# lajoiepy/cslam

Hardware: AMD Instinct MI355X
Metric: keyframes/sec (extract+match) on 100kx4096-D bank (higher is better)
Workload: dtype f32

## Files before the change

### cslam_amd/_lib.py

```python
import ctypes as C
import os
import subprocess

_HERE = os.path.dirname(os.path.abspath(__file__))
LIB_PATH = os.environ.get("CSLAM_HIP_LIB") or os.path.join(_HERE, "libcslam_hip.so")
CSRC_DIR = os.path.join(_HERE, "csrc")

F32, F64 = 0, 1
MODE_AUTO, MODE_SCAN, MODE_MFMA = 0, 1, 2


class CslamHipError(RuntimeError):
    pass


class CslamGraphError(CslamHipError):
    """CSLAM_E_GRAPH: the graph admits no Fiedler pair (not connected, singular junction Laplacian, TraceMIN breakdown) --
    the condition under which the reference's networkx call raises and acm.py:436-466 re-draws its start point.  Not a
    failure of the GPU path."""


class CslamUnsupportedError(CslamHipError):
    """CSLAM_E_UNSUPPORTED: an optional run-time dependency (RCCL, rocBLAS / rocSOLVER) was not found on this host."""

# ... 9 lines not shown
_vp, _i, _i64, _f = C.c_void_p, C.c_int, C.c_int64, C.c_float
_SIGNATURES = {
    "cslam_last_error": (C.c_char_p, []),
    "cslam_version": (_i, []),
    "cslam_device_count": (_i, [C.POINTER(_i)]),
    "cslam_device_info": (_i, [_i, C.c_char_p, _i, C.POINTER(_i64), C.POINTER(_i)]),
    "cslam_bank_create": (_i, [_i, _i, _i64, C.POINTER(_vp)]),
    "cslam_bank_destroy": (_i, [_vp]),
    "cslam_bank_size": (_i, [_vp, C.POINTER(_i64), C.POINTER(_i)]),
    "cslam_bank_clear": (_i, [_vp]),
    "cslam_bank_add_host": (_i, [_vp, _vp, _i, _i64]),
    "cslam_bank_add_dev": (_i, [_vp, _vp, _i64, _i64, _vp]),
    "cslam_bank_read_host": (_i, [_vp, _i64, _i64, _vp]),
    "cslam_bank_device_ptr": (_i, [_vp, C.POINTER(_vp), C.POINTER(_i64)]),
    "cslam_bank_search_host": (_i, [_vp, _vp, _i, _i64, _i, _vp, _i, _vp, _vp, _vp]),
    "cslam_bank_search_dev": (_i, [_vp, _vp, _i, _i64, _i64, _i, _vp, _i, _vp, _vp, _vp, _vp]),
    "cslam_bank_search_multi_dev": (_i, [_vp, _i, _vp, _i, _i64, _i64, _vp, _vp, _i, _vp, _vp, _vp, _vp]),
    "cslam_bank_search_enqueue_dev": (_i, [_vp, _vp, _i, _i64, _i64, _i, _vp, _i, _vp, _vp, _vp, _vp]),
    "cslam_bank_search_finish": (_i, [_vp, C.POINTER(_i64)]),
    "cslam_bank_search_flag_copy_dev": (_i, [_vp, _vp, _vp]),
    "cslam_bank_search_multi_enqueue_dev": (_i, [_vp, _i, _vp, _i, _i64, _i64, _vp, _vp, _i, _vp, _vp, _vp, _vp]),
    "cslam_bank_search_multi_finish": (_i, [_vp, _i, C.POINTER(_i64)]),
    "cslam_bank_last_stats": (_i, [_vp, C.POINTER(_i64 * 4)]),
    "cslam_bank_last_stage": (_i, [_vp, C.POINTER(C.c_int32 * 4)]),
    "cslam_bank_last_kernel_ms": (_i, [_vp, C.POINTER(_f)]),
    "cslam_topk_merge_dev": (_i, [_vp, _vp, _vp, _vp, _i, _i64, _i, _vp, _vp, _vp, _vp]),
    "cslam_l2_normalize_dev": (_i, [_vp, _i64, _i, _i64, _f, _i, _vp]),
    "cslam_vlad_aggregate_dev": (_i, [_vp, _vp, _vp, _vp, _i, _i, _i, _i, _vp, _i64, _vp]),
    "cslam_vlad_aggregate_nhwc_dev": (_i, [_vp, _vp, _vp, _vp, _i, _i, _i, _i, _vp, _i64, _vp]),
    "cslam_gem_fc_head_dev": (_i, [_vp, _f, _f, _vp, _vp, _i, _i, _i, _i, _vp, _vp]),
    "cslam_gem_fc_head_nhwc_dev": (_i, [_vp, _f, _f, _vp, _vp, _i, _i, _i, _i, _vp, _vp]),
    "cslam_pca_project_dev": (_i, [_vp, _i64, _vp, _i64, _vp, _vp, _i, _i, _i, _vp, _vp]),
    "cslam_pca_project_pairs_dev": (_i, [_vp, _i64, C.c_float, _vp, C.c_float, _i, _vp, _vp, _i, _i, _i, _vp, _vp]),
    "cslam_preprocess_dev": (_i, [_vp, _i, _i, _i, _i, _i, C.POINTER(_f * 3), C.POINTER(_f * 3), _vp, _vp]),
    "cslam_preprocess_nhwc_dev": (_i, [_vp, _i, _i, _i, _i, _i, C.POINTER(_f * 3), C.POINTER(_f * 3), _vp, _vp]),
    "cslam_mac_grad_dev": (_i, [_vp, _vp, _vp, _vp, _i64, _vp, _vp]),
    "cslam_csr_spmm_dev": (_i, [_vp, _vp, _vp, _i64, _vp, _i, _vp, _vp]),
    "cslam_csr_spmm4_dev": (_i, [_vp, _vp, _vp, _i64, _vp, _vp, _vp]),
    "cslam_block4_gram_dev": (_i, [_vp, _vp, _i64, _vp, _vp, _vp]),
    "cslam_block4_affine_dev": (_i, [_vp, _i64, _vp, _vp, _vp, _vp]),
    "cslam_block4_residual_dev": (_i, [_vp, _vp, _i64, _vp, C.c_double, _vp, _vp, _vp]),
    "cslam_block4_gram_sync": (_i, [_vp, _vp, _i64, _vp, _vp, _vp, _vp]),
    "cslam_block4_affine_host": (_i, [_vp, _i64, _vp, _vp, _vp, _vp]),
    "cslam_block4_residual_sync": (_i, [_vp, _vp, _i64, _vp, C.c_double, _vp, _vp, _vp, _vp]),
    "cslam_chain_forward_dev": (_i, [_vp, _vp, _vp, _i64, _vp, _i, _vp, _vp, _vp, _vp, _vp, _vp, _vp, _vp, _vp, _vp, _vp]),
    "cslam_chain_backward_dev": (_i, [_vp, _vp, _vp, _vp, _vp, _vp, _vp, _vp, _vp, _vp, _i64, _vp, _vp]),
    "cslam_chol_solve4_dev": (_i, [_vp, _i64, _i64, _i, _vp, _vp, _i, _vp, _vp, _vp]),
    "cslam_fiedler": (_i, [_i64, _vp, _vp, _vp, _vp, C.c_uint32, C.c_double, _i, _vp, _vp, _vp, _vp]),
    "cslam_fiedler_start_block": (_i, [C.c_uint32, _i64, _vp]),
    "cslam_fiedler_release": (_i, []),
    "cslam_mac_fw_subset": (_i, [_i64, _i64, _vp, _vp, _vp, _i64, _vp, _vp, _vp, _vp, _i64, _i, C.c_double, C.c_double, _vp, _vp, _vp, _vp, _vp]),
    "cslam_scbank_create": (_i, [_i, _i, _i, _i64, _vp]),
    "cslam_scbank_destroy": (_i, [_vp]),
    "cslam_scbank_size": (_i, [_vp, _vp, _vp, _vp]),
    "cslam_scbank_clear": (_i, [_vp]),
    "cslam_scbank_add_host": (_i, [_vp, _vp, _i64]),
    "cslam_scbank_add_dev": (_i, [_vp, _vp, _i64, _vp]),
    "cslam_scbank_read_host": (_i, [_vp, _i64, _i64, _vp, _vp]),
    "cslam_scbank_search_host": (_i, [_vp, _vp, _i64, _i, _vp, _vp, _vp, _vp, _vp, _vp, _vp]),
    "cslam_scbank_search_dev": (_i, [_vp, _vp, _i64, _i, _vp, _vp, _vp, _vp, _vp, _vp, _vp, _vp]),
    "cslam_bias_act_pool_dev": (_i, [_vp, _vp, _i, _i, _i, _i, _i, _i, _vp, _vp]),
    "cslam_conv3x3_c3_dev": (_i, [_vp, _vp, _vp, _i, _i, _i, _i, _i, _vp, _vp]),
    "cslam_wino_input_dev": (_i, [_vp, _i, _i, _i, _i, _vp, _vp]),
    "cslam_wino_output_dev": (_i, [_vp, _vp, _vp, _i, _i, _i, _i, _i, _i, _vp, _vp]),
    "cslam_wino4_input_dev": (_i, [_vp, _i, _i, _i, _i, _vp, _vp]),
    "cslam_wino4_output_dev": (_i, [_vp, _vp, _vp, _i, _i, _i, _i, _i, _i, _vp, _vp]),
    "cslam_absmax_dev": (_i, [_vp, _i64, _vp, _vp]),
    "cslam_wino4_input_h3_dev": (_i, [_vp, _i, _i, _i, _i, _vp, _vp, _vp]),
    "cslam_wino4_output_scaled_dev": (_i, [_vp, _vp, _vp, _i, _i, _i, _i, _i, _i, _vp, C.c_float, _vp, _vp, _vp]),
    "cslam_wino2_fused64_dev": (_i, [_vp, _vp, _vp, _i, _i, _i, _i, _i, _vp, _vp]),
    "cslam_wino2_fused_c64_dev": (_i, [_vp, _vp, _vp, _vp, _i, _i, _i, _i, _i, _i, _vp, _vp]),
    "cslam_wino4_fused_c64_dev": (_i, [_vp, _vp, _vp, _vp, _i, _i, _i, _i, _i, _i, _vp, _vp]),
    "cslam_scancontext_from_cloud_dev": (_i, [_vp, _vp, _i, _i, _i, C.c_double, _vp, _vp, _vp]),
    "cslam_wino4_fused_c64_h_dev": (_i, [_vp, _vp, _vp, _vp, _i, _i, _i, _i, _i, _i, _vp, C.c_float, _vp, _vp, _vp]),
    "cslam_conv3x3_direct_h_dev": (_i, [_vp, _vp, _vp, _i, _i, _i, _i, _i, _i, _i, _vp, _f, _vp, _vp, _vp]),
    "cslam_conv3x3_direct_r_dev": (_i, [_vp, _vp, _vp, _i, _i, _i, _i, _i, _i, _i, _vp, C.c_float, _vp, _vp, _vp]),
    "cslam_conv3x3_direct_r2_dev": (_i, [_vp, _vp, _vp, _i, _i, _i, _i, _i, _i, _i, _vp, C.c_float, _vp, _vp, _vp]),
    "cslam_conv_stem_direct_h_dev": (_i, [_vp, _vp, _vp, _vp, C.c_float, _vp, _vp, C.c_float, _i, _i, _i, _i, _vp, _vp, _vp, _vp]),
    "cslam_wino4_stem_c64_h_dev": (_i, [_vp, _vp, _vp, _vp, C.c_float, _vp, _vp, _i, _i, _i, _i, _vp, C.c_float, _vp, _vp, _vp]),
    "cslam_debug_wfh_prof_dev": (_i, [_vp]),
    "cslam_conv3x3_c3_amax_dev": (_i, [_vp, _vp, _vp, _i, _i, _i, _i, _i, _vp, _vp, _vp]),
    "cslam_wino4_input_h2_dev": (_i, [_vp, _i, _i, _i, _i, _vp, _vp, _vp]),
    "cslam_wino_gemm_h2_dev": (_i, [_vp, _vp, _i64, _i, _i, _vp, _vp]),
    "cslam_wino_zgemm_h2_dev": (_i, [_vp, _vp, _i64, _i, _i, _vp, _vp]),
    "cslam_wino4_output_z_dev": (_i, [_vp, _vp, _i, _i, _i, _i, _i, _i, _vp, C.c_float, _vp, _vp, _vp]),
    "cslam_conv_igemm_h2_dev": (_i, [_vp, _vp, _vp, _vp, _i, _i, _i, _i, _i, _i, _i, _i, _i, _i, _vp, C.c_float, _vp, _vp, _vp]),
    "cslam_conv_stem_pool_igemm_h2_dev": (_i, [_vp, _vp, _vp, _i, _i, _i, _i, _i, _i, _i, _i, _vp, C.c_float, _vp, _vp, _vp]),
    "cslam_conv_igemm_h2p_dev": (_i, [_vp, _i, _vp, _vp, _vp, _vp, _i, _vp, _i, _i, _i, _i, _i, _i, _i, _i, _i, _i, _vp, C.c_float,
                                      C.c_float, C.c_float, _vp, _i, _vp, _vp, _vp]),
    "cslam_conv3x3_direct_r_pairs_dev": (_i, [_vp, _vp, _vp, _i, _i, _i, _i, _i, _vp, C.c_float, C.c_float, C.c_float, _vp, _vp, _vp, _vp]),
    "cslam_conv3x3_direct_hp_dev": (_i, [_vp, _vp, _vp, _vp, _i, _i, _i, _i, _i, _i, _i, C.c_float, _vp, _vp, _vp]),
    "cslam_conv3x3_direct_p_dev": (_i, [_vp, _i, _vp, _vp, _vp, _vp, _i, _vp, _i, _i, _i, _i, _i, _i, _vp, C.c_float, C.c_float, C.c_float,
                                        _vp, _i, _vp, _vp, _vp]),
    "cslam_comm_unique_id": (_i, [_vp]),
    "cslam_comm_init": (_i, [_i, _i, _vp, _i, C.POINTER(_vp)]),
    "cslam_comm_destroy": (_i, [_vp]),
    "cslam_comm_info": (_i, [_vp, C.POINTER(_i), C.POINTER(_i)]),
    "cslam_allgather_queries_dev": (_i, [_vp, _vp, _i64, _i64, _vp, _vp]),
    "cslam_exchange_lists_dev": (_i, [_vp, _vp, _vp, _i64, _vp]),
    "cslam_peak_copy_dev": (_i, [_vp, _vp, _i64, _i, _vp]),
    "cslam_peak_mfma_dev": (_i, [_i, _i, _i, _i, _vp, C.POINTER(C.c_double), _vp]),
    "cslam_debug_last_candidates": (_i, [_vp, _i64, C.POINTER(_i), _vp, _vp, C.POINTER(C.c_double)]),
    "cslam_ring_schedule_describe": (_i, [_i, _i, _i, _i, C.POINTER(C.c_int32 * 6), _vp, _i64, _vp, _vp, _vp]),
    "cslam_trunk_timing": (_i, [_i]),
    "cslam_trunk_timing_read": (_i, [C.POINTER(C.c_double * 8)]),
}

EXPERIMENTAL_SYMBOLS = ("cslam_wino4_input_h3_dev", "cslam_wino2_fused64_dev", "cslam_wino2_fused_c64_dev",
                        "cslam_wino4_fused_c64_dev", "cslam_debug_wfh_prof_dev", "cslam_peak_copy_dev", "cslam_peak_mfma_dev",
                        "cslam_debug_last_candidates", "cslam_ring_schedule_describe", "cslam_trunk_timing", "cslam_trunk_timing_read")
EXPORTED_SYMBOLS = tuple(n for n in _SIGNATURES if n not in EXPERIMENTAL_SYMBOLS)


def build(verbose=False):
    r = subprocess.run(["make", "-C", CSRC_DIR, "-j", "4"], capture_output=True, text=True)
    if verbose or r.returncode != 0:
        print(r.stdout[-4000:])
        print(r.stderr[-4000:])
    if r.returncode != 0:
        raise CslamHipError("building libcslam_hip.so failed")
    return LIB_PATH


def load():
    global _lib
    if _lib is not None:
        return _lib
    try:
        import torch
    except ImportError:
        pass
    if not os.path.exists(LIB_PATH):
        raise CslamHipError(
            f"{LIB_PATH} not found: the HIP extension is not built "
            "(run `python __graft_entry__.py` or `make -C cslam_amd/csrc`); there is no CPU fallback")
    lib = C.CDLL(LIB_PATH)
    for name, (res, args) in _SIGNATURES.items():
        fn = getattr(lib, name)
        fn.restype = res
        fn.argtypes = args
    _lib = lib
    return lib


def check(rc):
    if rc != 0:
        msg = load().cslam_last_error()
        raise _ERROR_CLASSES.get(rc, CslamHipError)(f"libcslam_hip error {rc}: {msg.decode() if msg else ''}")


def require_gpu():
    lib = load()
    n = C.c_int(0)
    rc = lib.cslam_device_count(C.byref(n))
    if rc != 0 or n.value < 1:
        msg = lib.cslam_last_error()
        raise CslamHipError("no HIP device visible: cslam_amd needs an MI355X (gfx950); "
                            f"no CPU fallback exists ({msg.decode() if msg else ''})")
    return n.value
```

### cslam_amd/vpr/winograd.py

```python
import ctypes as C
import os

import torch
from torch import nn

from .. import _lib
from .heads import _p, _stream, pair_split

_G = torch.tensor([[1.0, 0.0, 0.0], [0.5, 0.5, 0.5], [0.5, -0.5, 0.5], [0.0, 0.0, 1.0]], dtype=torch.float64)
_G4 = torch.tensor([[1 / 4, 0.0, 0.0], [-1 / 6, -1 / 6, -1 / 6], [-1 / 6, 1 / 6, -1 / 6],
                    [1 / 24, 1 / 12, 1 / 6], [1 / 24, -1 / 12, 1 / 6], [0.0, 0.0, 1.0]], dtype=torch.float64)


def wino_weights(weight, tile=2):
    G = _G if tile == 2 else _G4
    g = weight.detach().to(torch.float64).cpu()
    u = torch.einsum("ik,ockl,jl->ijco", G, g, G)
    return u.reshape(G.shape[0] ** 2, g.shape[1], g.shape[0]).to(torch.float32).contiguous()


def split16_weights(U4):
    u = U4.detach().to(torch.float64)
    uh, ul, inv_su = pair_split(u)
    return torch.cat((uh, uh, ul), dim=1).contiguous(), inv_su
# ... 512 lines not shown
                self.blocks.append(d)
        return self

    @torch.no_grad()
    def __call__(self, x, x_bound=None):
        x = x.contiguous(memory_format=torch.channels_last)
        slots = self._buf("amax_slots", 4 * len(self.blocks) + 6, x.device)
        slots.zero_()
        nslot = [0]

        def fresh():
            nslot[0] += 1
            return slots[nslot[0] - 1:nslot[0]]

        def run(conv, inp, relu, res, a_in):
            out_slot = fresh()
            y = conv(self, inp, relu, res, a_in, out_slot)
            return y, (out_slot if self.amax_written else None)
        a0 = None
        if x_bound is not None:
            a0 = fresh()
            a0.fill_(float(x_bound))
        sp = self.stem_pool
        ho = (x.shape[2] + 2 * self.stem.padding[0] - self.stem.kernel[0]) // self.stem.stride[0] + 1
        wo = (x.shape[3] + 2 * self.stem.padding[1] - self.stem.kernel[1]) // self.stem.stride[1] + 1
        if (self.stem.Wg is not None and x.shape[1] == 3 and stem_pool_fits(ho, wo) and isinstance(sp, torch.nn.MaxPool2d)
                and _pair(sp.kernel_size) == (3, 3) and _pair(sp.stride) == (2, 2) and _pair(sp.padding) == (1, 1)
                and _pair(sp.dilation) == (1, 1) and not sp.ceil_mode):
            out_slot = fresh()
            x = self.stem(self, x, True, None, a0, out_slot, pool=True)
            ax = out_slot
        else:
            y, ax = run(self.stem, x, True, None, a0)
            x = sp(y)
        convs = [c for b in self.blocks for c in (b["down"], b["c1"], b["c2"], b["c3"]) if c is not None]
        if PAIR_ACTS and ax is not None and all(c.Wg is not None and c.in_channels % 32 == 0 for c in convs):
            pslots = self._buf("pair_slots", 2 * len(convs) + 2, x.device)
            pslots.zero_()
            np_ = [0]
            last = convs[-1]

            def runp(conv, a, relu, res):
                np_[0] += 2
                if (conv.Wp is not None and (a.pairs or res is None) and conv is not last
                        and direct_p_fits(conv.weight.shape, conv.kernel, conv.stride[0], conv.padding[0], a.shape[2], a.shape[3])):
                    return conv3x3_direct_p(a, conv.Wp, conv.bias, relu, res, conv.wl1, conv.bmax, pslots[np_[0] - 2:np_[0] - 1],
                                            pslots[np_[0] - 1:np_[0]], True)
                return conv_igemm_p(self, a, conv.Wg, conv.bias, conv.kernel, conv.stride[0], conv.padding[0], relu, res, conv.wl1,
                                    conv.bmax, pslots[np_[0] - 2:np_[0] - 1], pslots[np_[0] - 1:np_[0]], conv is not last)
            cur = PairAct(x, False, x.shape, ax, ax)
            for b in self.blocks:
                idt = cur if b["down"] is None else runp(b["down"], cur, False, None)
                o = runp(b["c1"], cur, True, None)
                if b["c3"] is None:
                    cur = runp(b["c2"], o, True, idt)
                else:
                    o = runp(b["c2"], o, True, None)
                    cur = runp(b["c3"], o, True, idt)
            return cur.t
        for b in self.blocks:
            idt = x if b["down"] is None else run(b["down"], x, False, None, ax)[0]
            o, ao = run(b["c1"], x, True, None, ax)
            if b["c3"] is None:
                x, ax = run(b["c2"], o, True, idt, ao)
            else:
                o, ao = run(b["c2"], o, True, None, ao)
                x, ax = run(b["c3"], o, True, idt, ao)
        return x


class _Step(object):
    __slots__ = ("kind", "module", "conv", "relu", "pool", "U", "U4", "U3", "U2", "Up", "Uph", "bias", "stem", "Wd", "Wr", "Wdr", "Wdr2", "wl1", "bmax")

    def __init__(self):
        self.kind, self.module, self.conv, self.relu, self.pool = "torch", None, None, False, False
        self.U, self.U4, self.U3, self.U2, self.Up, self.Uph, self.bias, self.stem = None, None, None, None, None, None, None, None
        self.Wd = None
        self.Wr = None
        self.Wdr = None
        self.Wdr2 = None
        self.wl1 = self.bmax = None


TRUNK_FORMS = {"conv_direct": 1, "conv_direct_r": True, "conv_direct_r2": True, "stem_direct": True, "wino_stem": True, "fused_h": True, "split16_min_cin": None}
FP32_GEMM_FORMS = {"split16_min_cin": 0, "fused_h": False, "wino_stem": False}


class WinogradTrunk(_Workspace):

    def __init__(self, encoder, min_in_channels=256, tile=2, fused64=None, split16_h3=False, forms=None):
        super().__init__()
        self.encoder = encoder
        self.min_in_channels = int(min_in_channels)
        self.tile = int(tile)
        self.fused64 = True if fused64 is None else bool(fused64)
        self.fused_min_blocks = 256
        self.fused_couts = (64, 128)
        self.input_bound = None
        self.forms = dict(TRUNK_FORMS)
        self.forms.update(forms or {})
        assert set(self.forms) == set(TRUNK_FORMS), "unknown trunk form"
        self.direct128 = int(self.forms["conv_direct"]) != 0
        self.direct_cins = (128,) if int(self.forms["conv_direct"]) == 2 else (64, 128)
        self.split16_h3 = bool(split16_h3)
        self.split16_min_cin = (256 if self.split16_h3 else 128) if self.forms["split16_min_cin"] is None else int(self.forms["split16_min_cin"])
        use_tuned_gemms()
        self.refresh()

    def refresh(self):
        mods = list(self.encoder)
        self.steps = []
        i = 0
        while i < len(mods):
            m = mods[i]
            st = _Step()
            ok = (isinstance(m, nn.Conv2d) and m.kernel_size == (3, 3) and m.stride == (1, 1) and m.padding == (1, 1)
                  and m.dilation == (1, 1) and m.groups == 1 and m.in_channels >= self.min_in_channels
                  and m.in_channels % 4 == 0 and m.out_channels % 4 == 0 and m.weight.is_cuda)
            if ok:
                st.kind, st.conv, st.relu, st.pool = "wino", m, False, False
                st.U = wino_weights(m.weight).to(m.weight.device)
                st.U4 = wino_weights(m.weight, 4).to(m.weight.device) if self.tile == 4 else None
                if st.U4 is not None and 0 < self.split16_min_cin <= m.in_channels:
                    if not self.split16_h3 and m.in_channels % 32 == 0 and m.out_channels % 128 == 0:
                        st.U2 = split16_pair_weights(st.U4)
                    else:
                        st.U3 = split16_weights(st.U4)
                if self.fused64 and m.in_channels == 64 and m.out_channels in self.fused_couts:
                    t4 = self.tile == 4
                    st.Up = fused64_weights(st.U4 if t4 else st.U)
                    if t4 and self.forms["fused_h"]:
                        st.Uph = fused64_pair_weights(st.U4)
                if (self.direct128 and self.tile == 4 and m.out_channels == 128 and m.in_channels in self.direct_cins):
                    st.Wd = direct_pair_weights(m.weight)
                    if m.in_channels == 64 and self.forms["conv_direct_r"]:
                        st.Wdr = direct_r_pair_weights(m.weight)
                        st.wl1 = float(m.weight.detach().abs().sum(dim=(1, 2, 3)).max())
                        st.bmax = 0.0 if m.bias is None else float(m.bias.detach().abs().max())
                    if m.in_channels == 128 and self.forms.get("conv_direct_r2", True):
                        st.Wdr2 = direct_r2_pair_weights(m.weight)
                st.bias = None if m.bias is None else m.bias.detach().to(torch.float32).contiguous()
                i += 1
                if i < len(mods) and isinstance(mods[i], nn.ReLU):
                    st.relu = True
                    i += 1
                    p = mods[i] if i < len(mods) else None
                    if isinstance(p, nn.MaxPool2d) and p.kernel_size in (2, (2, 2)) and p.stride in (2, (2, 2)) \
                            and p.padding in (0, (0, 0)) and not p.ceil_mode:
                        st.pool = True
                        i += 1
            elif (isinstance(m, nn.Conv2d) and m.in_channels == 3 and m.kernel_size == (3, 3) and m.stride == (1, 1)
                  and m.padding == (1, 1) and m.dilation == (1, 1) and m.groups == 1 and m.out_channels % 16 == 0
                  and m.out_channels <= 512 and m.weight.is_cuda and not (i + 2 < len(mods) and isinstance(
                      mods[i + 1], nn.ReLU) and isinstance(mods[i + 2], nn.MaxPool2d))):
                st.kind, st.conv = "c3", m
                st.U = m.weight.detach().to(torch.float32).permute(1, 2, 3, 0).reshape(27, m.out_channels).contiguous()
                st.bias = None if m.bias is None else m.bias.detach().to(torch.float32).contiguous()
                i += 1
                if i < len(mods) and isinstance(mods[i], nn.ReLU):
                    st.relu = True
                    i += 1
            elif (isinstance(m, nn.Conv2d) and m.groups == 1 and m.out_channels % 4 == 0 and m.bias is not None
                  and m.weight.is_cuda and i + 1 < len(mods) and isinstance(mods[i + 1], nn.ReLU)):
                st.kind, st.conv, st.relu = "direct", m, True
                st.bias = m.bias.detach().to(torch.float32).contiguous()
                i += 2
                p = mods[i] if i < len(mods) else None
                if isinstance(p, nn.MaxPool2d) and p.kernel_size in (2, (2, 2)) and p.stride in (2, (2, 2)) \
                        and p.padding in (0, (0, 0)) and not p.ceil_mode:
                    st.pool = True
                    i += 1
            else:
                st.kind, st.module = "torch", m
                i += 1
            self.steps.append(st)
        if self.forms["wino_stem"]:
            for a, b in zip(self.steps, self.steps[1:]):
                if (a.kind == "c3" and a.relu and a.conv.out_channels == 64 and b.kind == "wino" and b.Uph is not None
                        and b.relu and b.conv.out_channels == 64):
                    a.stem = stem_pair_weights(a.conv.weight)
                    if self.forms["stem_direct"]:
                        a.Wr = stem_direct_pair_weights(b.conv.weight)
        return self

    @torch.no_grad()
    def __call__(self, x):
        lib = _lib.load()
        slots = amax_ready = None
        wants = lambda st_: st_ is not None and (st_.U3 is not None or st_.U2 is not None or st_.Uph is not None or st_.Wd is not None)
        if any(wants(st) for st in self.steps):
            slots = self._buf("amax_slots", len(self.steps) + 1, x.device)
            slots.zero_()
        skip = False
        for k, st in enumerate(self.steps):
            if skip:
                skip = False
                continue
            have, amax_ready = amax_ready, None
            nxt = self.steps[k + 1] if k + 1 < len(self.steps) else None
            if st.kind == "c3":
                x = x.contiguous()
                B, _, H, W = x.shape
                if (st.stem is not None and B * -(-H // 16) * -(-W // 16) >= self.fused_min_blocks
                        and not (nxt.pool and (H % 2 or W % 2)) and B * H * W * 64 < 2 ** 31):
                    slot = slots[k:k + 1]
                    if self.input_bound is not None:
                        slot.fill_(float(self.input_bound))
                    elif x.numel() % 4 == 0:
                        _lib.check(lib.cslam_absmax_dev(_p(x), x.numel(), _p(slot), _stream(x)))
                    else:
                        slot.copy_(x.abs().max().reshape(1))
                    nn2 = self.steps[k + 2] if k + 2 < len(self.steps) else None
                    want = slots[k + 2:k + 3] if wants(nn2) else None
                    if st.Wr is not None:
                        x = conv_stem_direct_h(x, st.stem, st.bias, st.Wr, nxt.bias, nxt.pool, slot, want)
                    else:
                        x = wino_stem64_h(x, st.stem, st.bias, nxt.Uph, nxt.bias, nxt.pool, slot, want)
                    amax_ready = want is not None
                    skip = True
                    continue
                Cout = st.conv.out_channels
                y = torch.empty((B, Cout, H, W), dtype=torch.float32, device=x.device, memory_format=torch.channels_last)
                want = slots[k + 1:k + 2] if (wants(nxt) and Cout == 64) else None
                _lib.check(lib.cslam_conv3x3_c3_amax_dev(_p(x), _p(st.U), _p(st.bias) if st.bias is not None else None,
                                                         B, H, W, Cout, int(st.relu), _p(y),
                                                         _p(want) if want is not None else None, _stream(x)))
                amax_ready = want is not None
                x = y
                continue
            x = x.contiguous(memory_format=torch.channels_last)
            if st.kind == "torch":
                x = st.module(x)
                continue
            if st.kind == "direct":
                c = st.conv
                x = torch.nn.functional.conv2d(x, c.weight, None, c.stride, c.padding, c.dilation)
                x = x.contiguous(memory_format=torch.channels_last)
                B, Cout, H, W = x.shape
                pool = st.pool and H % 2 == 0 and W % 2 == 0
                y = x if not pool else torch.empty((B, Cout, H // 2, W // 2), dtype=torch.float32, device=x.device,
                                                   memory_format=torch.channels_last)
                _lib.check(lib.cslam_bias_act_pool_dev(_p(x), _p(st.bias), B, H, W, Cout, 1, int(pool), _p(y), _stream(x)))
                x = y if not (st.pool and not pool) else torch.nn.functional.max_pool2d(y, 2, 2)
                continue
            x = x.contiguous(memory_format=torch.channels_last)
            if (st.Wd is not None and not (st.pool and (x.shape[2] % 2 or x.shape[3] % 2))
                    and x.shape[0] * -(-x.shape[2] // 16) * -(-x.shape[3] // 16) >= self.fused_min_blocks and x.numel() % 4 == 0):
                slot = slots[k:k + 1]
                if not have:
                    _lib.check(lib.cslam_absmax_dev(_p(x), x.numel(), _p(slot), _stream(x)))
                want = slots[k + 1:k + 2] if wants(nxt) else None
                if (VGG_PAIRS and st.Wdr is not None and st.relu and not st.pool and nxt is not None and nxt.Wd is not None
                        and nxt.Wdr is None and nxt.conv.in_channels == 128 and x.shape[2] * x.shape[3] * 512 < 2 ** 31 - 16
                        and not (nxt.pool and (x.shape[2] % 2 or x.shape[3] % 2))):
                    B_, _, H_, W_ = x.shape
                    bslot = self._buf("vgg_pair_bound", 1, x.device)
                    w_ = st.conv.weight.detach()
                    xp = conv3x3_direct_r_pairs(x, st.Wdr, st.bias, float(w_.abs().sum(dim=(1, 2, 3)).max()) if st.wl1 is None else st.wl1,
                                                0.0 if st.bias is None else st.bmax, slot, bslot)
                    nn2 = self.steps[k + 2] if k + 2 < len(self.steps) else None
                    want2 = slots[k + 2:k + 3] if wants(nn2) else None
                    x = conv3x3_direct_hp(xp, (B_, 128, H_, W_), bslot, nxt.Wd, nxt.bias, nxt.relu, nxt.pool, want2)
                    amax_ready = want2 is not None
                    skip = True
                    continue
                if st.Wdr is not None and x.shape[2] * x.shape[3] * 512 < 2 ** 31 - 16:
                    x = conv3x3_direct_r(x, st.Wdr, st.bias, st.relu, st.pool, slot, want)
                elif st.Wdr2 is not None and x.shape[2] * x.shape[3] * 512 < 2 ** 31 - 16:
                    x = conv3x3_direct_r2(x, st.Wdr2, st.bias, st.relu, st.pool, slot, want)
                else:
                    x = conv3x3_direct_h(x, st.Wd, st.bias, st.relu, st.pool, slot, want)
                amax_ready = want is not None
                continue
            if st.Up is not None and not (st.pool and (x.shape[2] % 2 or x.shape[3] % 2)):
                bh, bw = (16, 16) if st.Up.shape[1] == 36 else (8, 16)
                nblk = x.shape[0] * -(-x.shape[2] // bh) * -(-x.shape[3] // bw) * st.Up.shape[2] // 4
                if nblk >= self.fused_min_blocks:
                    if st.Uph is not None and x.numel() < 2 ** 31:
                        slot = slots[k:k + 1]
                        if not have:
                            _lib.check(lib.cslam_absmax_dev(_p(x), x.numel(), _p(slot), _stream(x)))
                        want = slots[k + 1:k + 2] if wants(nxt) else None
                        x = wino_fused64_h(x, st.Uph, st.bias, st.relu, st.pool, slot, want)
                        amax_ready = want is not None
                    else:
                        x = wino_fused64(x, st.Up, st.bias, st.relu, st.pool)
                    continue
            want = slots[k + 1:k + 2] if wants(nxt) else None
            y = wino_conv3x3(self, x, st.U, st.U4, st.bias, st.relu, st.pool, U3=st.U3, U2=st.U2,
                             amax_in=slots[k:k + 1] if have else None, amax_out=want)
            amax_ready = want is not None and self.amax_written
            x = y
        return x
```

### include/cslam_hip.h

```cpp
#ifndef CSLAM_HIP_H
#define CSLAM_HIP_H

#include <stdint.h>

#ifdef __cplusplus
extern "C" {
#endif

#define CSLAM_OK 0
#define CSLAM_E_INVALID (-1)
#define CSLAM_E_HIP (-2)
#define CSLAM_E_NOMEM (-3)
#define CSLAM_E_DIM (-4)
#define CSLAM_E_UNSUPPORTED (-5)
#define CSLAM_E_GRAPH (-6)
#define CSLAM_E_LIMIT (-7)

#define CSLAM_F32 0
#define CSLAM_F64 1

#define CSLAM_MODE_AUTO 0
#define CSLAM_MODE_SCAN 1
#define CSLAM_MODE_MFMA 2

// ... 70 lines not shown

int cslam_mac_grad_dev(const double *d_fiedler, const int32_t *d_edge_i, const int32_t *d_edge_j,
                       const double *d_weights, int64_t m, double *d_grad, void *stream);
int cslam_csr_spmm_dev(const int64_t *d_indptr, const int32_t *d_indices, const double *d_data,
                       int64_t n, const double *d_x, int nvec, double *d_y, void *stream);

int cslam_csr_spmm4_dev(const int64_t *d_indptr, const int32_t *d_indices, const double *d_data,
                        int64_t n, const double *d_x, double *d_y, void *stream);

int cslam_block4_gram_dev(const double *d_A, const double *d_B, int64_t n, double *d_partial,
                          double *d_out20, void *stream);
int cslam_block4_affine_dev(const double *d_A, int64_t n, const double *d_M16, const double *d_shift4,
                            double *d_out, void *stream);
int cslam_block4_residual_dev(const double *d_W, const double *d_X, int64_t n, const double *d_y4,
                              double sigma, double *d_partial, double *d_out1, void *stream);

int cslam_block4_gram_sync(const double *d_A, const double *d_B, int64_t n, double *d_partial, double *d_out20,
                           double *h_out20, void *stream);
int cslam_block4_affine_host(const double *d_A, int64_t n, const double *h_M16, const double *h_shift4, double *d_out,
                             void *stream);
int cslam_block4_residual_sync(const double *d_W, const double *d_X, int64_t n, const double *h_y4, double sigma,
                               double *d_partial, double *d_out1, double *h_out1, void *stream);

int cslam_chain_forward_dev(const double *d_b, const uint8_t *d_is_junction, const double *d_r, int64_t n,
                            const int64_t *d_J, int nJ, const int *d_seg_start_of, const int *d_seg_end_of,
                            const int64_t *d_sa, const int64_t *d_sb, const double *d_Rl,
                            double *d_Bn, double *d_Qn, double *d_tmp, double *d_scratch, double *d_bt,
                            void *stream);
int cslam_chain_backward_dev(const double *d_xJ, const double *d_Bn, const double *d_Qn, const double *d_r,
                             const double *d_Rn, const int *d_jid, const int *d_seg_of, const int64_t *d_sa,
                             const int64_t *d_sb, const double *d_Rl, int64_t n, double *d_x, void *stream);
int cslam_chol_solve4_dev(const double *d_L, int64_t m, int64_t ld, int col_major, const double *d_dinv,
                          const double *d_dinvT, int bs, double *d_x, double *d_tmp, void *stream);

int cslam_fiedler(int64_t n, const int64_t *h_indptr, const int32_t *h_indices, const double *h_data, const double *h_x0,
                  uint32_t seed, double tol, int max_iters, double *h_lambda2, double *h_v, int *h_iters, void *stream);
int cslam_fiedler_start_block(uint32_t seed, int64_t n, double *h_x0);
int cslam_fiedler_release(void);

int cslam_mac_fw_subset(int64_t num_poses, int64_t n_fixed, const int64_t *fixed_i, const int64_t *fixed_j,
                        const double *fixed_w, int64_t n_cand, const int64_t *cand_i, const int64_t *cand_j,
                        const double *cand_w, const double *w_init, int64_t k, int max_iters, double duality_gap_tol,
                        double fiedler_tol, double *h_selected, double *h_w_unrounded, double *h_upper, int *h_iters,
                        void *stream);

typedef struct cslam_scbank cslam_scbank_t;
int cslam_scbank_create(int device, int rings, int sectors, int64_t capacity_hint, cslam_scbank_t **out);
int cslam_scbank_destroy(cslam_scbank_t *bank);
int cslam_scbank_size(const cslam_scbank_t *bank, int64_t *n, int *rings, int *sectors);
int cslam_scbank_clear(cslam_scbank_t *bank);
int cslam_scbank_add_host(cslam_scbank_t *bank, const double *sc, int64_t n);
int cslam_scbank_add_dev(cslam_scbank_t *bank, const double *d_sc, int64_t n, void *stream);
int cslam_scbank_read_host(const cslam_scbank_t *bank, int64_t first, int64_t count, double *sc_out,
                           double *ringkeys_out);
int cslam_scbank_search_host(cslam_scbank_t *bank, const double *queries, int64_t nq, int num_candidates,
                             const int64_t *row_limit, int64_t *best_idx, double *best_sim,
                             int32_t *best_yaw, int64_t *cand, double *cdist, int32_t *cyaw);
int cslam_scbank_search_dev(cslam_scbank_t *bank, const double *d_queries, int64_t nq, int num_candidates,
                            const int64_t *d_row_limit, int64_t *d_best_idx, double *d_best_sim,
                            int32_t *d_best_yaw, int64_t *d_cand, double *d_cdist, int32_t *d_cyaw,
                            void *stream);

int cslam_scancontext_from_cloud_dev(const double *d_points, const int64_t *d_offsets, int n_frames,
                                     int rings, int sectors, double max_length, double *d_out,
                                     int32_t *d_status, void *stream);

int cslam_bias_act_pool_dev(const float *d_x, const float *d_bias, int B, int H, int W, int C, int relu,
                            int pool, float *d_y, void *stream);
int cslam_conv3x3_c3_dev(const float *d_x, const float *d_wt, const float *d_bias, int B, int H, int W,
                         int Cout, int relu, float *d_y, void *stream);
int cslam_wino_input_dev(const float *d_x, int B, int H, int W, int C, float *d_V, void *stream);
int cslam_wino_output_dev(const float *d_M, const float *d_bias, const float *d_residual, int B, int H, int W,
                          int C, int relu, int pool, float *d_y, void *stream);
int cslam_wino4_input_dev(const float *d_x, int B, int H, int W, int C, float *d_V, void *stream);
int cslam_wino4_output_dev(const float *d_M, const float *d_bias, const float *d_residual, int B, int H, int W,
                           int C, int relu, int pool, float *d_y, void *stream);
int cslam_absmax_dev(const float *d_x, int64_t n, unsigned *d_slot, void *stream);
int cslam_wino4_output_scaled_dev(const float *d_M, const float *d_bias, const float *d_residual, int B, int H, int W,
                                  int C, int relu, int pool, const unsigned *d_amax, float inv_su, unsigned *d_amax_out,
                                  float *d_y, void *stream);
int cslam_wino4_input_h2_dev(const float *d_x, int B, int H, int W, int C, const unsigned *d_amax, void *d_V2,
                             void *stream);
int cslam_wino_gemm_h2_dev(const void *d_V2, const void *d_U2, int64_t T, int Cin, int Cout, float *d_M, void *stream);
int cslam_wino_zgemm_h2_dev(const void *d_V2, const void *d_U2, int64_t T, int Cin, int Cout, float *d_Z, void *stream);
int cslam_wino4_output_z_dev(const float *d_Z, const float *d_bias, int B, int H, int W, int C, int relu, int pool,
                             const unsigned *d_amax, float inv_su, unsigned *d_amax_out, float *d_y, void *stream);

int cslam_wino4_fused_c64_h_dev(const float *d_x, const void *d_Uh, const float *d_bias, const float *d_residual, int B,
                                int H, int W, int Cout, int relu, int pool, const unsigned *d_amax, float inv_su,
                                unsigned *d_amax_out, float *d_y, void *stream);
int cslam_conv3x3_direct_h_dev(const float *d_x, const void *d_w2, const float *d_bias, int B, int H, int W, int Cin, int Cout,
                               int relu, int pool, const unsigned *d_amax, float inv_sw, unsigned *d_amax_out, float *d_y,
                               void *stream);
int cslam_conv3x3_c3_amax_dev(const float *d_x, const float *d_wt, const float *d_bias, int B, int H, int W, int Cout,
                              int relu, float *d_y, unsigned *d_amax_out, void *stream);

int cslam_wino4_stem_c64_h_dev(const float *d_x0, const void *d_w1, const float *d_b1, const float *d_sumw, float inv_sw,
                               const void *d_Uh, const float *d_bias, int B, int H, int W, int pool,
                               const unsigned *d_amax_x0, float inv_su, unsigned *d_amax_out, float *d_y, void *stream);

int cslam_conv_igemm_h2_dev(const float *d_x, const void *d_w2, const float *d_bias, const float *d_res, int B, int H, int W,
                            int Cin, int Cout, int KH, int KW, int stride, int pad, int relu, const unsigned *d_amax_in,
                            float inv_sw, unsigned *d_amax_out, float *d_y, void *stream);
int cslam_conv_stem_pool_igemm_h2_dev(const float *d_x, const void *d_w2, const float *d_bias, int B, int H, int W, int Cout,
                                      int KH, int KW, int stride, int pad, const unsigned *d_amax_in, float inv_sw,
                                      unsigned *d_amax_out, float *d_y, void *stream);
int cslam_conv_igemm_h2p_dev(const void *d_x, int x_pairs, const unsigned *d_xbound, const void *d_w2, const float *d_bias,
                             const void *d_res, int res_pairs, const unsigned *d_res_bound, int B, int H, int W, int Cin,
                             int Cout, int KH, int KW, int stride, int pad, int relu, const unsigned *d_amax_in, float inv_sw,
                             float wl1, float bmax, unsigned *d_amax_out, int out_pairs, unsigned *d_bound_out, void *d_y,
                             void *stream);

int cslam_conv3x3_direct_r_dev(const float *d_x, const void *d_w2r, const float *d_bias, int B, int H, int W, int Cin, int Cout,
                               int relu, int pool, const unsigned *d_amax, float inv_sw, unsigned *d_amax_out, float *d_y,
                               void *stream);

int cslam_conv3x3_direct_r2_dev(const float *d_x, const void *d_w2r2, const float *d_bias, int B, int H, int W, int Cin, int Cout,
                                int relu, int pool, const unsigned *d_amax, float inv_sw, unsigned *d_amax_out, float *d_y,
                                void *stream);

int cslam_conv3x3_direct_r_pairs_dev(const float *d_x, const void *d_w2r, const float *d_bias, int B, int H, int W, int Cin, int Cout,
                                     const unsigned *d_amax, float inv_sw, float wl1, float bmax, unsigned *d_amax_out,
                                     unsigned *d_bound_out, void *d_y, void *stream);
int cslam_conv3x3_direct_hp_dev(const void *d_x, const unsigned *d_xbound, const void *d_w2, const float *d_bias, int B, int H, int W,
                                int Cin, int Cout, int relu, int pool, float inv_sw, unsigned *d_amax_out, float *d_y, void *stream);

int cslam_conv3x3_direct_p_dev(const void *d_x, int x_pairs, const unsigned *d_xbound, const void *d_w2r, const float *d_bias, const void *d_res,
                               int res_pairs, const unsigned *d_res_bound, int B, int H, int W, int Cin, int Cout, int relu,
                               const unsigned *d_amax_in, float inv_sw, float wl1, float bmax, unsigned *d_amax_out, int out_pairs,
                               unsigned *d_bound_out, void *d_y, void *stream);

int cslam_conv_stem_direct_h_dev(const float *d_x0, const void *d_w1, const float *d_b1, const float *d_sumw, float inv_sw1,
                                 const void *d_w2r, const float *d_bias, float inv_sw2, int B, int H, int W, int pool,
                                 const unsigned *d_amax_x0, unsigned *d_amax_out, float *d_y, void *stream);

int cslam_comm_unique_id(void *id128);
int cslam_comm_init(int world, int rank, const void *id128, int device, cslam_comm_t **out);
int cslam_comm_destroy(cslam_comm_t *comm);
int cslam_comm_info(const cslam_comm_t *comm, int *world, int *rank);
int cslam_allgather_queries_dev(cslam_comm_t *comm, const void *d_local, int64_t rows, int64_t row_bytes, void *d_all,
                                void *stream);
int cslam_exchange_lists_dev(cslam_comm_t *comm, const void *d_send, void *d_recv, int64_t bytes_per_rank, void *stream);

#ifdef __cplusplus
}
#endif
#endif
```

Measured before the change: 17690.

## Chain consecutive Winograd F(4,3) convs without materialising intermediate activations

Adds a fused kernel that takes one layer's Winograd-domain GEMM output and does the inverse transform, bias, ReLU, and the next layer's input transform plus split-fp16 packing in one pass. It keeps a ring of output rows in LDS, so the intermediate activation map never goes to global memory. The per-layer absmax pass is replaced by an analytic bound (input amax times weight L1 plus bias max). This removes a round trip to global memory and a reduction launch per chained layer. The bound is looser than a true absmax, which may cost fp16 precision, and the kernel adds LDS and register pressure.

```diff
diff --git a/cslam_amd/_lib.py b/cslam_amd/_lib.py
--- a/cslam_amd/_lib.py
+++ b/cslam_amd/_lib.py
@@ -115,6 +115,7 @@
     "cslam_conv3x3_c3_amax_dev": (_i, [_vp, _vp, _vp, _i, _i, _i, _i, _i, _vp, _vp, _vp]),
     "cslam_wino4_input_h2_dev": (_i, [_vp, _i, _i, _i, _i, _vp, _vp, _vp]),
     "cslam_wino_gemm_h2_dev": (_i, [_vp, _vp, _i64, _i, _i, _vp, _vp]),
+    "cslam_wino4_chain_h2_dev": (_i, [_vp, _vp, _i, _i, _i, _i, _vp, C.c_float, _vp, C.c_float, C.c_float, _vp, _vp, _vp, _vp]),
     "cslam_wino_zgemm_h2_dev": (_i, [_vp, _vp, _i64, _i, _i, _vp, _vp]),
     "cslam_wino4_output_z_dev": (_i, [_vp, _vp, _i, _i, _i, _i, _i, _i, _vp, C.c_float, _vp, _vp, _vp]),
     "cslam_conv_igemm_h2_dev": (_i, [_vp, _vp, _vp, _vp, _i, _i, _i, _i, _i, _i, _i, _i, _i, _i, _vp, C.c_float, _vp, _vp, _vp]),
diff --git a/cslam_amd/csrc/wino_chain.hip b/cslam_amd/csrc/wino_chain.hip
--- /dev/null
+++ b/cslam_amd/csrc/wino_chain.hip
@@ -0,0 +1,215 @@
+#include "common.h"
+#include "pairs.h"
+#include <hip/hip_fp16.h>
+
+typedef float cf4 __attribute__((ext_vector_type(4)));
+typedef unsigned cu2 __attribute__((ext_vector_type(2)));
+typedef unsigned cu4 __attribute__((ext_vector_type(4)));
+
+__device__ __forceinline__ void wc_at4(const cf4 m0, const cf4 m1, const cf4 m2, const cf4 m3, const cf4 m4, const cf4 m5,
+                                       cf4 &s0, cf4 &s1, cf4 &s2, cf4 &s3) {
+    const cf4 a = m1 + m2, bq = m1 - m2, c = m3 + m4, e = m3 - m4;
+    s0 = m0 + a + c;
+    s1 = bq + 2.0f * e;
+    s2 = a + 4.0f * c;
+    s3 = bq + 8.0f * e + m5;
+}
+__device__ __forceinline__ void wc_bt4(cf4 &d0, cf4 &d1, cf4 &d2, cf4 &d3, cf4 &d4, cf4 &d5) {
+    const cf4 r0 = 4.0f * d0 - 5.0f * d2 + d4;
+    const cf4 r1 = -4.0f * (d1 + d2) + d3 + d4;
+    const cf4 r2 = 4.0f * (d1 - d2) - d3 + d4;
+    const cf4 r3 = 2.0f * (d3 - d1) - d2 + d4;
+    const cf4 r4 = 2.0f * (d1 - d3) - d2 + d4;
+    const cf4 r5 = 4.0f * d1 - 5.0f * d3 + d5;
+    d0 = r0; d1 = r1; d2 = r2; d3 = r3; d4 = r4; d5 = r5;
+}
+
+#define WC_THREADS 128
+#define WC_RING 9
+
+struct WcArgs {
+    const float *mb;
+    __half *vb;
+    unsigned moff, voff;
+    float *rp;
+    int64_t mplane, vplane, mrow, vrow;
+    int H, TH, Wr, tj;
+    float inv, sc;
+    cf4 bv;
+    cf4 clim;
+    bool odd;
+};
+
+template <int CG, bool OUT, bool LOAD, bool IN>
+__device__ __forceinline__ void wc_step(const WcArgs &a, const int r, cf4 (&m)[36], float &vmax) {
+    if (OUT) {
+        cf4 s[4][6];
+#pragma unroll
+        for (int j = 0; j < 6; ++j)
+            wc_at4(m[j], m[6 + j], m[12 + j], m[18 + j], m[24 + j], m[30 + j], s[0][j], s[1][j], s[2][j], s[3][j]);
+#pragma unroll
+        for (int i = 0; i < 4; ++i) {
+            cf4 o[4];
+            wc_at4(s[i][0], s[i][1], s[i][2], s[i][3], s[i][4], s[i][5], o[0], o[1], o[2], o[3]);
+            const int h = 4 * r + i;
+            float *row = a.rp + ((h % WC_RING) * a.Wr + 4 * a.tj) * CG;
+            const cf4 lim = h < a.H ? a.clim : (cf4)(0.0f);
+#pragma unroll
+            for (int j = 0; j < 4; ++j) {
+                cf4 v = __builtin_elementwise_max(o[j] * a.inv + a.bv, (cf4)(0.0f));
+                v = __builtin_elementwise_min(v, (cf4)(lim[j]));
+                vmax = fmaxf(fmaxf(vmax, fmaxf(v.x, v.y)), fmaxf(v.z, v.w));
+                *(cf4 *)(row + j * CG) = v;
+            }
+        }
+    }
+    __syncthreads();
+    if (LOAD) {
+        const float *p = a.mb + (r + 1) * a.mrow;
+#pragma unroll
+        for (int q = 0; q < 36; ++q) m[q] = __builtin_nontemporal_load((const cf4 *)(p + q * a.mplane + a.moff));
+    }
+    if (IN) {
+        const int h0 = 4 * (r - 1) - 1, w0 = 4 * a.tj - 1;
+        const int Hr = 4 * a.TH;
+        cf4 d[6][6];
+#pragma unroll
+        for (int i = 0; i < 6; ++i) {
+            const int hh = h0 + i;
+            const float *row = a.rp + ((hh + WC_RING) % WC_RING) * a.Wr * CG;
+#pragma unroll
+            for (int j = 0; j < 6; ++j) {
+                const int ww = w0 + j;
+                const bool in = (hh >= 0) & (hh < Hr) & (ww >= 0) & (ww < a.Wr);
+                cf4 v = *(const cf4 *)(row + (j == 0 ? max(ww, 0) : j == 5 ? min(ww, a.Wr - 1) : ww) * CG);
+                asm("" : "+v"(v));
+                d[i][j] = in ? v * a.sc : (cf4)(0.0f);
+            }
+        }
+#pragma unroll
+        for (int j = 0; j < 6; ++j) wc_bt4(d[0][j], d[1][j], d[2][j], d[3][j], d[4][j], d[5][j]);
+#pragma unroll
+        for (int i = 0; i < 6; ++i) wc_bt4(d[i][0], d[i][1], d[i][2], d[i][3], d[i][4], d[i][5]);
+        __half *o = a.vb + (r - 1) * a.vrow;
+#pragma unroll
+        for (int i = 0; i < 6; ++i)
+#pragma unroll
+            for (int j = 0; j < 6; ++j) {
+                const cf4 v = d[i][j];
+                const __half2 h0v = __floats2half2_rn(v.x, v.y), h1v = __floats2half2_rn(v.z, v.w);
+                const __half2 l0v = __floats2half2_rn(sub_half<0>(v.x, h0v), sub_half<1>(v.y, h0v));
+                const __half2 l1v = __floats2half2_rn(sub_half<0>(v.z, h1v), sub_half<1>(v.w, h1v));
+                cu2 hi, lo;
+                hi.x = *(const unsigned *)&h0v; hi.y = *(const unsigned *)&h1v;
+                lo.x = *(const unsigned *)&l0v; lo.y = *(const unsigned *)&l1v;
+                const cu2 give = a.odd ? hi : lo;
+                cu2 got;
+                got.x = (unsigned)__builtin_amdgcn_mov_dpp((int)give.x, 0xB1, 0xF, 0xF, true);
+                got.y = (unsigned)__builtin_amdgcn_mov_dpp((int)give.y, 0xB1, 0xF, 0xF, true);
+                cu4 v16;
+                if (a.odd) { v16.x = got.x; v16.y = got.y; v16.z = lo.x; v16.w = lo.y; }
+                else { v16.x = hi.x; v16.y = hi.y; v16.z = got.x; v16.w = got.y; }
+                __builtin_nontemporal_store(v16, (cu4 *)(o + (6 * i + j) * a.vplane + a.voff));
+            }
+    }
+    __syncthreads();
+}
+
+template <int CG>
+__global__ __launch_bounds__(WC_THREADS) void wino4_chain_h2_kernel(const float *__restrict__ M, const float *__restrict__ bias,
+                                                                     int B, int H, int W, int C,
+                                                                     const unsigned *__restrict__ vscale, float inv_su,
+                                                                     const unsigned *__restrict__ amax_x, float wl1, float bmax,
+                                                                     unsigned *__restrict__ amax_out,
+                                                                     unsigned *__restrict__ bound_out, __half *__restrict__ V2) {
+    extern __shared__ __attribute__((aligned(16))) float ring[];
+    __shared__ unsigned wg_amax;
+    constexpr int C4G = CG / 4;
+    WcArgs a;
+    a.H = H;
+    a.TH = (H + 3) >> 2;
+    const int TW = (W + 3) >> 2;
+    a.Wr = 4 * TW;
+    const int ncg = C / CG;
+    const int b = blockIdx.x / ncg, cg = blockIdx.x - b * ncg;
+    a.tj = threadIdx.x / C4G;
+    const int c4 = threadIdx.x % C4G;
+    const int c = cg * CG + 4 * c4;
+    const int64_t T = (int64_t)B * a.TH * TW;
+    const int64_t t0 = (int64_t)b * a.TH * TW;
+    if (threadIdx.x == 0) wg_amax = 0u;
+
+    a.inv = inv_su / scale_le_327_68(__uint_as_float(*vscale));
+    const float bound = fmaf(__uint_as_float(*amax_x), wl1, bmax);
+    a.sc = scale_le_327_68(bound);
+    if (blockIdx.x == 0 && threadIdx.x == 0) *bound_out = __float_as_uint(bound);
+    a.bv = bias ? *(const cf4 *)(bias + c) : (cf4)(0.0f);
+#pragma unroll
+    for (int j = 0; j < 4; ++j) a.clim[j] = 4 * a.tj + j < W ? __builtin_inff() : 0.0f;
+    a.odd = threadIdx.x & 1;
+    a.mplane = T * C;
+    a.vplane = T * 2 * C;
+    a.mrow = (int64_t)TW * C;
+    a.vrow = (int64_t)TW * 2 * C;
+    a.mb = M + t0 * C + cg * CG;
+    a.vb = V2 + t0 * 2 * C + cg * 2 * CG;
+    a.moff = a.tj * C + 4 * c4;
+    a.voff = a.tj * 2 * C + (c4 >> 3) * 64 + (4 * c4 & 31) + (a.odd ? 32 - 4 : 0);
+    a.rp = ring + 4 * c4;
+    float vmax = 0.0f;
+
+    cf4 m[36];
+#pragma unroll
+    for (int q = 0; q < 36; ++q) m[q] = __builtin_nontemporal_load((const cf4 *)(a.mb + q * a.mplane + a.moff));
+    const int TH = a.TH;
+    if (TH == 1) {
+        wc_step<CG, true, false, false>(a, 0, m, vmax);
+    } else {
+        wc_step<CG, true, true, false>(a, 0, m, vmax);
+#pragma unroll 1
+        for (int r = 1; r < TH - 1; ++r) wc_step<CG, true, true, true>(a, r, m, vmax);
+        wc_step<CG, true, false, true>(a, TH - 1, m, vmax);
+    }
+    wc_step<CG, false, false, true>(a, TH, m, vmax);
+#pragma unroll
+    for (int o = 32; o > 0; o >>= 1) vmax = fmaxf(vmax, __shfl_xor(vmax, o, 64));
+    if ((threadIdx.x & 63) == 0) atomicMax(&wg_amax, __float_as_uint(vmax));
+    __syncthreads();
+    if (threadIdx.x == 0 && wg_amax > *(volatile unsigned *)amax_out) atomicMax(amax_out, wg_amax);
+}
+
+template <int CG>
+static int wino4_chain_launch(const float *d_M, const float *d_bias, int B, int H, int W, int C, const unsigned *d_vscale,
+                              float inv_su, const unsigned *d_amax_x, float wl1, float bmax, unsigned *d_amax_out,
+                              unsigned *d_bound_out, void *d_V2, void *stream) {
+    const size_t lds = (size_t)WC_RING * 4 * ((W + 3) / 4) * CG * sizeof(float);
+    ARG_CHECK(lds <= 144 * 1024, "map too wide for the LDS ring");
+    static DeviceOnce once;
+    int dev;
+    if (once.todo(&dev)) {
+        HIP_TRY(hipFuncSetAttribute((const void *)wino4_chain_h2_kernel<CG>, hipFuncAttributeMaxDynamicSharedMemorySize, 144 * 1024));
+        once.done(dev);
+    }
+    hipLaunchKernelGGL(wino4_chain_h2_kernel<CG>, dim3((unsigned)((int64_t)B * (C / CG))), dim3(((W + 3) / 4) * (CG / 4)), lds, (hipStream_t)stream,
+                       d_M, d_bias, B, H, W, C, d_vscale, inv_su, d_amax_x, wl1, bmax, d_amax_out, d_bound_out, (__half *)d_V2);
+    HIP_TRY(hipGetLastError());
+    return CSLAM_OK;
+}
+
+CSLAM_API int cslam_wino4_chain_h2_dev(const float *d_M, const float *d_bias, int B, int H, int W, int C,
+                                       const unsigned *d_vscale, float inv_su, const unsigned *d_amax_x, float wl1, float bmax,
+                                       unsigned *d_amax_out, unsigned *d_bound_out, void *d_V2, void *stream) {
+    PTR_DEVICE(d_M);
+    ARG_CHECK(d_M && d_V2 && d_vscale && d_amax_x && d_amax_out && d_bound_out, "NULL argument");
+    ARG_CHECK(B >= 1 && H >= 1 && W >= 1, "empty map");
+    ARG_CHECK(C >= 32 && (C % 32) == 0, "C must be a multiple of 32");
+    ARG_CHECK(inv_su > 0.0f && wl1 >= 0.0f && bmax >= 0.0f, "inv_su must be positive, wl1 and bmax non-negative");
+    const int TW = (W + 3) / 4;
+    ARG_CHECK(TW <= 16, "maps wider than 64 pixels stay on the separate transforms");
+    ARG_CHECK((int64_t)B * (C / 32) < (1LL << 31), "too many frames for one launch");
+    if (TW <= 4 && (C % 128) == 0)
+        return wino4_chain_launch<128>(d_M, d_bias, B, H, W, C, d_vscale, inv_su, d_amax_x, wl1, bmax, d_amax_out, d_bound_out, d_V2, stream);
+    if (TW <= 8 && (C % 64) == 0)
+        return wino4_chain_launch<64>(d_M, d_bias, B, H, W, C, d_vscale, inv_su, d_amax_x, wl1, bmax, d_amax_out, d_bound_out, d_V2, stream);
+    return wino4_chain_launch<32>(d_M, d_bias, B, H, W, C, d_vscale, inv_su, d_amax_x, wl1, bmax, d_amax_out, d_bound_out, d_V2, stream);
+}
diff --git a/cslam_amd/vpr/winograd.py b/cslam_amd/vpr/winograd.py
--- a/cslam_amd/vpr/winograd.py
+++ b/cslam_amd/vpr/winograd.py
@@ -618,7 +618,9 @@
         self.wl1 = self.bmax = None
 
 
-TRUNK_FORMS = {"conv_direct": 1, "conv_direct_r": True, "conv_direct_r2": True, "stem_direct": True, "wino_stem": True, "fused_h": True, "split16_min_cin": None}
+TRUNK_FORMS = {"conv_direct": 1, "conv_direct_r": True, "conv_direct_r2": True, "stem_direct": True, "wino_stem": True, "fused_h": True, "split16_min_cin": None,
+               "wino_chain": True}
+CHAIN_TILE_COLS = (5, 16)
 FP32_GEMM_FORMS = {"split16_min_cin": 0, "fused_h": False, "wino_stem": False}
 
 
@@ -676,6 +678,9 @@
                     if m.in_channels == 128 and self.forms.get("conv_direct_r2", True):
                         st.Wdr2 = direct_r2_pair_weights(m.weight)
                 st.bias = None if m.bias is None else m.bias.detach().to(torch.float32).contiguous()
+                if st.U2 is not None and st.wl1 is None:
+                    st.wl1 = float(m.weight.detach().abs().sum(dim=(1, 2, 3)).max())
+                    st.bmax = 0.0 if m.bias is None else float(m.bias.detach().abs().max())
                 i += 1
                 if i < len(mods) and isinstance(mods[i], nn.ReLU):
                     st.relu = True
@@ -719,6 +724,47 @@
                         a.Wr = stem_direct_pair_weights(b.conv.weight)
         return self
 
+    def _chain_len(self, k, B, H, W):
+        t4h, t4w = -(-H // 4), -(-W // 4)
+        if not (self.forms["wino_chain"] and B * t4h * t4w >= 512 and 16 * t4h * t4w <= 1.35 * H * W
+                and CHAIN_TILE_COLS[0] <= t4w <= CHAIN_TILE_COLS[1]):
+            return 1
+        pair = lambda st_: (st_.kind == "wino" and st_.U2 is not None and st_.Wd is None and st_.Up is None
+                            and not _z_form(st_.conv.in_channels, st_.conv.out_channels))
+        n = 1
+        while (k + n < len(self.steps) and pair(self.steps[k + n - 1]) and pair(self.steps[k + n])
+               and self.steps[k + n - 1].relu and not self.steps[k + n - 1].pool):
+            n += 1
+        return n
+
+    def _run_chain(self, x, k, n, have, slots, want):
+        lib = _lib.load()
+        B, Cin, H, W = x.shape
+        T = B * -(-H // 4) * -(-W // 4)
+        s = _stream(x)
+        if not have:
+            _lib.check(lib.cslam_absmax_dev(_p(x), x.numel(), _p(slots[k:k + 1]), s))
+        bounds = self._buf("chain_bounds", len(self.steps) + 1, x.device)
+        V2 = self._buf("V", 36 * T * Cin, x.device)
+        _lib.check(lib.cslam_wino4_input_h2_dev(_p(x), B, H, W, Cin, _p(slots[k:k + 1]), _p(V2), s))
+        vscale = slots[k:k + 1]
+        for j in range(k, k + n):
+            st = self.steps[j]
+            Cin, Cout = st.conv.in_channels, st.conv.out_channels
+            M = self._buf("M", 36 * T * Cout, x.device)
+            _lib.check(lib.cslam_wino_gemm_h2_dev(_p(V2), _p(st.U2[0]), T, Cin, Cout, _p(M), s))
+            bias = _p(st.bias) if st.bias is not None else None
+            if j + 1 < k + n:
+                V2 = self._buf("V", 36 * T * Cout, x.device)
+                _lib.check(lib.cslam_wino4_chain_h2_dev(_p(M), bias, B, H, W, Cout, _p(vscale), float(st.U2[1]), _p(slots[j:j + 1]),
+                                                        st.wl1, st.bmax, _p(slots[j + 1:j + 2]), _p(bounds[j + 1:j + 2]), _p(V2), s))
+                vscale = bounds[j + 1:j + 2]
+        Ho, Wo = (H // 2, W // 2) if st.pool else (H, W)
+        y = torch.empty((B, Cout, Ho, Wo), dtype=torch.float32, device=x.device, memory_format=torch.channels_last)
+        _lib.check(lib.cslam_wino4_output_scaled_dev(_p(M), bias, None, B, H, W, Cout, int(st.relu), int(st.pool), _p(vscale), float(st.U2[1]),
+                                                     _p(want) if want is not None else None, _p(y), s))
+        return y
+
     @torch.no_grad()
     def __call__(self, x):
         lib = _lib.load()
@@ -727,10 +773,10 @@
         if any(wants(st) for st in self.steps):
             slots = self._buf("amax_slots", len(self.steps) + 1, x.device)
             slots.zero_()
-        skip = False
+        skip = 0
         for k, st in enumerate(self.steps):
             if skip:
-                skip = False
+                skip -= 1
                 continue
             have, amax_ready = amax_ready, None
             nxt = self.steps[k + 1] if k + 1 < len(self.steps) else None
@@ -753,7 +799,7 @@
                     else:
                         x = wino_stem64_h(x, st.stem, st.bias, nxt.Uph, nxt.bias, nxt.pool, slot, want)
                     amax_ready = want is not None
-                    skip = True
+                    skip = 1
                     continue
                 Cout = st.conv.out_channels
                 y = torch.empty((B, Cout, H, W), dtype=torch.float32, device=x.device, memory_format=torch.channels_last)
@@ -798,7 +844,7 @@
                     want2 = slots[k + 2:k + 3] if wants(nn2) else None
                     x = conv3x3_direct_hp(xp, (B_, 128, H_, W_), bslot, nxt.Wd, nxt.bias, nxt.relu, nxt.pool, want2)
                     amax_ready = want2 is not None
-                    skip = True
+                    skip = 1
                     continue
                 if st.Wdr is not None and x.shape[2] * x.shape[3] * 512 < 2 ** 31 - 16:
                     x = conv3x3_direct_r(x, st.Wdr, st.bias, st.relu, st.pool, slot, want)
@@ -822,6 +868,14 @@
                     else:
                         x = wino_fused64(x, st.Up, st.bias, st.relu, st.pool)
                     continue
+            n = self._chain_len(k, x.shape[0], x.shape[2], x.shape[3])
+            if n > 1:
+                after = self.steps[k + n] if k + n < len(self.steps) else None
+                want = slots[k + n:k + n + 1] if wants(after) else None
+                x = self._run_chain(x, k, n, have, slots, want)
+                amax_ready = want is not None
+                skip = n - 1
+                continue
             want = slots[k + 1:k + 2] if wants(nxt) else None
             y = wino_conv3x3(self, x, st.U, st.U4, st.bias, st.relu, st.pool, U3=st.U3, U2=st.U2,
                              amax_in=slots[k:k + 1] if have else None, amax_out=want)
diff --git a/include/cslam_hip.h b/include/cslam_hip.h
--- a/include/cslam_hip.h
+++ b/include/cslam_hip.h
@@ -176,6 +176,9 @@
 int cslam_wino4_input_h2_dev(const float *d_x, int B, int H, int W, int C, const unsigned *d_amax, void *d_V2,
                              void *stream);
 int cslam_wino_gemm_h2_dev(const void *d_V2, const void *d_U2, int64_t T, int Cin, int Cout, float *d_M, void *stream);
+int cslam_wino4_chain_h2_dev(const float *d_M, const float *d_bias, int B, int H, int W, int C, const unsigned *d_vscale,
+                             float inv_su, const unsigned *d_amax_x, float wl1, float bmax, unsigned *d_amax_out,
+                             unsigned *d_bound_out, void *d_V2, void *stream);
 int cslam_wino_zgemm_h2_dev(const void *d_V2, const void *d_U2, int64_t T, int Cin, int Cout, float *d_Z, void *stream);
 int cslam_wino4_output_z_dev(const float *d_Z, const float *d_bias, int B, int H, int W, int C, int relu, int pool,
                              const unsigned *d_amax, float inv_su, unsigned *d_amax_out, float *d_y, void *stream);
```

After: 18500 (median of 6 runs). 4.5% higher.
